# dexmal/dexbotic

Hardware: AMD Instinct MI355X
Metric: episodes/sec DB-CogACT fine-tune (higher is better)
Workload: dtype bf16; 1 GPU; DB-CogACT fine-tune step (CLIP-L/14@224 x1 view, Qwen2.5-7B-class 28L decoder, DiT-B head, AdamW), 16 episodes/GPU, 32-token instruction, S=287; global_batch=16, seq_len=287, parallelism=dp1, optimizer=AdamW serial, grad_accum=1, activations=resident

## Files before the change

dexbotic_amd/csrc/norm.hip:

```cpp
#include <stdlib.h>

#include "common.h"

namespace {

template <typename T, typename TW, int VEC>
__global__ __launch_bounds__(256) void rmsnorm_fwd_k(const T* __restrict__ x, const TW* __restrict__ w,
                                                     T* __restrict__ y, float* __restrict__ rstd_out,
                                                     int64_t rows, int64_t cols, float eps) {
  const int lane = threadIdx.x & 63;
  const int64_t row = (int64_t)blockIdx.x * 4 + (threadIdx.x >> 6);
  if (row >= rows) return;
  const T* xr = x + row * cols;
  float ss = 0.f;
  for (int64_t c = (int64_t)lane * VEC; c < cols; c += 64 * VEC) {
    float v[VEC];
    Vec<T, VEC>::ld(v, xr + c);
#pragma unroll
    for (int i = 0; i < VEC; ++i) ss += v[i] * v[i];
  }
  ss = wave_sum(ss);
  const float rstd = rsqrtf(ss / (float)cols + eps);
  if (lane == 0 && rstd_out) rstd_out[row] = rstd;
  T* yr = y + row * cols;
// ... 192 lines not shown
    if (slab) {
      for (int turn = 0; turn < 4; ++turn) {
        if (turn == wave && ok) {
          const T* xr = x + row * cols;
          const T* x2r = ADD ? x2 + row * cols : nullptr;
          const T* gr = dy + row * cols;
          for (int64_t c = (int64_t)lane * VEC; c < cols; c += 64 * VEC) {
            float xv[VEC], gv[VEC];
            ld_row<T, VEC, ADD>(xv, xr, x2r, c);
            Vec<T, VEC>::ld(gv, gr + c);
#pragma unroll
            for (int i = 0; i < VEC; ++i) {
              slab[c + i] += gv[i] * ((xv[i] - mu) * rs);
              slab[cols + c + i] += gv[i];
            }
          }
        }
        __syncthreads();
      }
    }
  }
}

template <typename T, bool DIRECT = false>
__global__ __launch_bounds__(256) void colsum_stage1_k(const T* __restrict__ x, int64_t ld, float* __restrict__ part,
                                                       int64_t rows, int64_t cols, int vec, int accumulate = 0) {
  __shared__ float red[4][256];
  const int lane = threadIdx.x & 63, wave = threadIdx.x >> 6;
  const int64_t c0 = (int64_t)blockIdx.x * 256 + lane * 4;
  const int64_t per = (rows + gridDim.y - 1) / gridDim.y;
  const int64_t r0 = (int64_t)blockIdx.y * per, r1 = min(rows, r0 + per);
  float a[4] = {0.f, 0.f, 0.f, 0.f};
  if (c0 < cols) {
    const int n_ok = (int)min((int64_t)4, cols - c0);
    for (int64_t r = r0 + wave; r < r1; r += 4) {
      const T* p = x + r * ld + c0;
      if (vec && n_ok == 4) {
        float v[4];
        Vec<T, 4>::ld(v, p);
#pragma unroll
        for (int i = 0; i < 4; ++i) a[i] += v[i];
      } else {
        for (int i = 0; i < n_ok; ++i) a[i] += ldf<T>(p + i);
      }
    }
  }
#pragma unroll
  for (int i = 0; i < 4; ++i) red[wave][lane * 4 + i] = a[i];
  __syncthreads();
  const int t = threadIdx.x;
  const int64_t c = (int64_t)blockIdx.x * 256 + t;
  if (c < cols) {
    const float sum = red[0][t] + red[1][t] + red[2][t] + red[3][t];
    if (DIRECT) part[c] = accumulate ? part[c] + sum : sum;
    else part[(int64_t)blockIdx.y * cols + c] = sum;
  }
}
__global__ void colsum_stage2_k(const float* __restrict__ part, float* __restrict__ out, int nsplit, int64_t cols,
                                int accumulate) {
  const int64_t c = (int64_t)blockIdx.x * blockDim.x + threadIdx.x;
  if (c >= cols) return;
  float s = 0.f;
  int i = 0;
  for (; i + 8 <= nsplit; i += 8) {
    float v[8];
#pragma unroll
    for (int u = 0; u < 8; ++u) v[u] = part[(int64_t)(i + u) * cols + c];
#pragma unroll
    for (int u = 0; u < 8; ++u) s += v[u];
  }
  for (; i < nsplit; ++i) s += part[(int64_t)i * cols + c];
  out[c] = accumulate ? out[c] + s : s;
}

template <typename T>
__global__ __launch_bounds__(256) void colsum_fused_k(const T* __restrict__ x, int64_t ld, float* __restrict__ part,
                                                      float* __restrict__ out, int64_t rows, int64_t cols, int vec,
                                                      int accumulate, int* __restrict__ cnt) {
  __shared__ float red[4][256];
  __shared__ int last;
  const int lane = threadIdx.x & 63, wave = threadIdx.x >> 6;
  const int64_t c0 = (int64_t)blockIdx.x * 256 + lane * 4;
  const int64_t per = (rows + gridDim.y - 1) / gridDim.y;
  const int64_t r0 = (int64_t)blockIdx.y * per, r1 = min(rows, r0 + per);
  float a[4] = {0.f, 0.f, 0.f, 0.f};
  if (c0 < cols) {
    const int n_ok = (int)min((int64_t)4, cols - c0);
    for (int64_t r = r0 + wave; r < r1; r += 4) {
      const T* p = x + r * ld + c0;
      if (vec && n_ok == 4) {
        float v[4];
        Vec<T, 4>::ld(v, p);
#pragma unroll
        for (int i = 0; i < 4; ++i) a[i] += v[i];
      } else {
        for (int i = 0; i < n_ok; ++i) a[i] += ldf<T>(p + i);
      }
    }
  }
#pragma unroll
  for (int i = 0; i < 4; ++i) red[wave][lane * 4 + i] = a[i];
  __syncthreads();
  const int t = threadIdx.x;
  const int64_t c = (int64_t)blockIdx.x * 256 + t;
  if (c < cols)
    __hip_atomic_store(part + (int64_t)blockIdx.y * cols + c, red[0][t] + red[1][t] + red[2][t] + red[3][t], __ATOMIC_RELAXED,
                       __HIP_MEMORY_SCOPE_AGENT);
  asm volatile("s_waitcnt vmcnt(0)" ::: "memory");
  __syncthreads();
  if (t == 0) {
    const int arrived = __hip_atomic_fetch_add(cnt + blockIdx.x, 1, __ATOMIC_RELAXED, __HIP_MEMORY_SCOPE_AGENT) + 1;
    last = arrived == (int)gridDim.y;
    if (last) __hip_atomic_store(cnt + blockIdx.x, 0, __ATOMIC_RELAXED, __HIP_MEMORY_SCOPE_AGENT);
  }
  __syncthreads();
  if (!last || c >= cols) return;
  const int nsplit = (int)gridDim.y;
  float s = 0.f;
  int i = 0;
  for (; i + 8 <= nsplit; i += 8) {
    float v[8];
#pragma unroll
    for (int u = 0; u < 8; ++u) v[u] = __hip_atomic_load(part + (int64_t)(i + u) * cols + c, __ATOMIC_RELAXED, __HIP_MEMORY_SCOPE_AGENT);
#pragma unroll
    for (int u = 0; u < 8; ++u) s += v[u];
  }
  for (; i < nsplit; ++i) s += __hip_atomic_load(part + (int64_t)i * cols + c, __ATOMIC_RELAXED, __HIP_MEMORY_SCOPE_AGENT);
  out[c] = accumulate ? out[c] + s : s;
}

inline bool al16(const void* p) { return (reinterpret_cast<uintptr_t>(p) & 15) == 0; }
inline bool al8(const void* p) { return (reinterpret_cast<uintptr_t>(p) & 7) == 0; }

template <typename T, typename TW, bool LN>
__global__ __launch_bounds__(256) void norm_bwd_fast_k(const T* __restrict__ dy, const T* __restrict__ x,
                                                       const TW* __restrict__ w, const float* __restrict__ mean,
                                                       const float* __restrict__ rstd, T* __restrict__ dx,
                                                       const T* __restrict__ res, float* __restrict__ partial,
                                                       int64_t rows, int64_t cols) {
  constexpr int NIT = 16;
  const int lane = threadIdx.x & 63, wave = threadIdx.x >> 6;
  const int64_t prow = (int64_t)blockIdx.x * 4 + wave;
  float aw[NIT][4], ab[NIT][4];
#pragma unroll
  for (int it = 0; it < NIT; ++it)
#pragma unroll
    for (int i = 0; i < 4; ++i) { aw[it][i] = 0.f; ab[it][i] = 0.f; }
  for (int64_t row = prow; row < rows; row += (int64_t)gridDim.x * 4) {
    const float rs = rstd[row];
    const float mu = LN ? mean[row] : 0.f;
    const T* xr = x + row * cols;
// ... 64 lines not shown
          }
        }
      }
      __syncthreads();
    }
    if (wave == 0) {
      float* pr = partial + (int64_t)blockIdx.x * (LN ? 2 : 1) * cols;
#pragma unroll
      for (int it = 0; it < NIT; ++it) {
        const int64_t c = ((int64_t)it * 64 + lane) * 4;
        if (c < cols) {
          const float4 t = *reinterpret_cast<const float4*>(sh + c);
          *reinterpret_cast<float4*>(pr + c) = make_float4(t.x + aw[it][0], t.y + aw[it][1], t.z + aw[it][2], t.w + aw[it][3]);
          if (LN) {
            const float4 u = *reinterpret_cast<const float4*>(sh + cols + c);
            *reinterpret_cast<float4*>(pr + cols + c) = make_float4(u.x + ab[it][0], u.y + ab[it][1], u.z + ab[it][2], u.w + ab[it][3]);
          }
        }
      }
    }
  }
}

template <typename TW, bool LN>
__global__ __launch_bounds__(256) void norm_bwd_fast8_k(const bf16_t* __restrict__ dy, const bf16_t* __restrict__ x,
                                                        const TW* __restrict__ w, const float* __restrict__ mean,
                                                        const float* __restrict__ rstd, bf16_t* __restrict__ dx,
                                                        const bf16_t* __restrict__ res, float* __restrict__ partial,
                                                        int64_t rows, int64_t cols) {
  constexpr int NIT = 8;
  typedef uint32_t u32x4 __attribute__((ext_vector_type(4)));
  const int lane = threadIdx.x & 63, wave = threadIdx.x >> 6;
  const int64_t prow = (int64_t)blockIdx.x * 4 + wave;
  float aw[NIT][8], ab[LN ? NIT : 1][8];
#pragma unroll
  for (int it = 0; it < NIT; ++it)
#pragma unroll
    for (int i = 0; i < 8; ++i) { aw[it][i] = 0.f; if (LN) ab[it][i] = 0.f; }
  auto unpack = [](const u32x4& v, float (&o)[8]) {
#pragma unroll
    for (int e = 0; e < 4; ++e) { o[2 * e] = __uint_as_float(v[e] << 16); o[2 * e + 1] = __uint_as_float(v[e] & 0xffff0000u); }
  };
  for (int64_t row = prow; row < rows; row += (int64_t)gridDim.x * 4) {
    const float rs = rstd[row];
    const float mu = LN ? mean[row] : 0.f;
    const bf16_t* xr = x + row * cols;
    const bf16_t* gr = dy + row * cols;
    u32x4 xv[NIT], gv[NIT];
#pragma unroll
    for (int it = 0; it < NIT; ++it) {
      const int64_t c = ((int64_t)it * 64 + lane) * 8;
      xv[it] = c < cols ? *reinterpret_cast<const u32x4*>(xr + c) : (u32x4){0u, 0u, 0u, 0u};
      gv[it] = c < cols ? *reinterpret_cast<const u32x4*>(gr + c) : (u32x4){0u, 0u, 0u, 0u};
    }
    float s1 = 0.f, s2 = 0.f;
#pragma unroll
    for (int it = 0; it < NIT; ++it) {
      const int64_t c = ((int64_t)it * 64 + lane) * 8;
      if (c < cols) {
        float xf[8], gf[8], w0[4] = {1.f, 1.f, 1.f, 1.f}, w1[4] = {1.f, 1.f, 1.f, 1.f};
        unpack(xv[it], xf); unpack(gv[it], gf);
        if (w) { Vec<TW, 4>::ld(w0, w + c); Vec<TW, 4>::ld(w1, w + c + 4); }
#pragma unroll
        for (int i = 0; i < 8; ++i) {
          const float g = gf[i] * (i < 4 ? w0[i] : w1[i - 4]);
          s1 += g;
          s2 += g * ((xf[i] - mu) * rs);
        }
      }
    }
    const float c1 = LN ? wave_sum(s1) / (float)cols : 0.f;
    const float c2 = wave_sum(s2) / (float)cols;
    bf16_t* dxr = dx + row * cols;
#pragma unroll
    for (int it = 0; it < NIT; ++it) {
      const int64_t c = ((int64_t)it * 64 + lane) * 8;
      if (c < cols) {
        float xf[8], gf[8], o[8], w0[4] = {1.f, 1.f, 1.f, 1.f}, w1[4] = {1.f, 1.f, 1.f, 1.f};
        unpack(xv[it], xf); unpack(gv[it], gf);
        if (w) { Vec<TW, 4>::ld(w0, w + c); Vec<TW, 4>::ld(w1, w + c + 4); }
#pragma unroll
        for (int i = 0; i < 8; ++i) {
          const float xh = (xf[i] - mu) * rs;
          o[i] = rs * (gf[i] * (i < 4 ? w0[i] : w1[i - 4]) - c1 - xh * c2);
          aw[it][i] += gf[i] * (LN ? xh : rnd<bf16_t>(xh));
          if (LN) ab[it][i] += gf[i];
        }
        if (res) {
          float rf[8];
          unpack(*reinterpret_cast<const u32x4*>(res + row * cols + c), rf);
#pragma unroll
          for (int i = 0; i < 8; ++i) o[i] += rf[i];
        }
        u32x4 ov;
#pragma unroll
        for (int e = 0; e < 4; ++e) ov[e] = pack_bf16x2(o[2 * e], o[2 * e + 1]);
        *reinterpret_cast<u32x4*>(dxr + c) = ov;
      }
    }
  }
  if (partial) {
    __shared__ float sh[(LN ? 2 : 1) * 4096];
    for (int turn = 3; turn >= 1; --turn) {
      if (wave == turn) {
#pragma unroll
        for (int it = 0; it < NIT; ++it) {
          const int64_t c = ((int64_t)it * 64 + lane) * 8;
          if (c < cols) {
#pragma unroll
            for (int i = 0; i < 8; ++i) {
              sh[c + i] = turn == 3 ? aw[it][i] : sh[c + i] + aw[it][i];
              if (LN) sh[cols + c + i] = turn == 3 ? ab[it][i] : sh[cols + c + i] + ab[it][i];
            }
          }
        }
      }
      __syncthreads();
    }
    if (wave == 0) {
      float* pr = partial + (int64_t)blockIdx.x * (LN ? 2 : 1) * cols;
#pragma unroll
      for (int it = 0; it < NIT; ++it) {
        const int64_t c = ((int64_t)it * 64 + lane) * 8;
        if (c < cols) {
#pragma unroll
// ... 119 lines not shown
      }
    }
  }
}

constexpr int NORM_BWD_MAX_BLOCKS = 512;
constexpr int64_t NORM_BWD_FAST_MAX_COLS = 4096;

template <bool LN>
bool launch_norm_bwd_fast(const void* dy, const void* x, const void* w, const float* mean, const float* rstd, void* dx,
                          const void* res, float* partial, int64_t rows, int64_t cols, int dtype, int w_dtype, bool vec_ok, hipStream_t st) {
  int64_t g = (rows + 3) / 4;
  if (g > NORM_BWD_MAX_BLOCKS) g = NORM_BWD_MAX_BLOCKS;
  dim3 grid((unsigned)g);
  if (!LN && vec_ok && dtype == DXA_BF16 && cols % 16 == 0 && cols <= 8192 && (cols * 4) % 16 == 0 &&
      (!partial || (reinterpret_cast<uintptr_t>(partial) & 15) == 0)) {
#define LAUNCH_SPLIT(TW_, NIT_, NS_) hipLaunchKernelGGL((rmsnorm_bwd_split_k<TW_, NIT_, NS_>), grid, dim3(NS_ * 128), 0, st, (const bf16_t*)dy, (const bf16_t*)x, (const TW_*)w, rstd, (bf16_t*)dx, (const bf16_t*)res, partial, rows, cols)
    if (w_dtype == DXA_BF16) { if (cols > 4096) LAUNCH_SPLIT(bf16_t, 8, 4); else LAUNCH_SPLIT(bf16_t, 4, 4); }
    else { if (cols > 4096) LAUNCH_SPLIT(float, 8, 4); else LAUNCH_SPLIT(float, 4, 4); }
#undef LAUNCH_SPLIT
    return true;
  }
  if (!vec_ok || cols % 4 != 0 || cols > NORM_BWD_FAST_MAX_COLS) return false;
  if (dtype == DXA_BF16 && cols % 8 == 0 && !LN) {
    if (w_dtype == DXA_BF16)
      hipLaunchKernelGGL((norm_bwd_fast8_k<bf16_t, LN>), grid, dim3(256), 0, st, (const bf16_t*)dy, (const bf16_t*)x, (const bf16_t*)w, mean, rstd, (bf16_t*)dx, (const bf16_t*)res, partial, rows, cols);
    else
      hipLaunchKernelGGL((norm_bwd_fast8_k<float, LN>), grid, dim3(256), 0, st, (const bf16_t*)dy, (const bf16_t*)x, (const float*)w, mean, rstd, (bf16_t*)dx, (const bf16_t*)res, partial, rows, cols);
    return true;
  }
  if (dtype == DXA_BF16 && w_dtype == DXA_BF16)
    hipLaunchKernelGGL((norm_bwd_fast_k<bf16_t, bf16_t, LN>), grid, dim3(256), 0, st, (const bf16_t*)dy, (const bf16_t*)x, (const bf16_t*)w, mean, rstd, (bf16_t*)dx, (const bf16_t*)res, partial, rows, cols);
  else if (dtype == DXA_BF16)
    hipLaunchKernelGGL((norm_bwd_fast_k<bf16_t, float, LN>), grid, dim3(256), 0, st, (const bf16_t*)dy, (const bf16_t*)x, (const float*)w, mean, rstd, (bf16_t*)dx, (const bf16_t*)res, partial, rows, cols);
  else
    hipLaunchKernelGGL((norm_bwd_fast_k<float, float, LN>), grid, dim3(256), 0, st, (const float*)dy, (const float*)x, (const float*)w, mean, rstd, (float*)dx, (const float*)res, partial, rows, cols);
  return true;
}

}

extern "C" int dxa_norm_bwd_blocks(int64_t rows) {
  int64_t g = (rows + 3) / 4;
  if (g < 1) g = 1;
  if (g > NORM_BWD_MAX_BLOCKS) g = NORM_BWD_MAX_BLOCKS;
  return (int)g;
}

static int check_norm_dtypes(int dtype, int w_dtype, const char* who) {
  if (!(dtype == DXA_F32 || dtype == DXA_BF16) || !(w_dtype == DXA_F32 || w_dtype == DXA_BF16) ||
      (dtype == DXA_F32 && w_dtype == DXA_BF16)) {
// ... 32 lines not shown
  const float rstd = rsqrtf(ss / (float)cols + eps);
  if (lane == 0 && rstd_out) rstd_out[row] = rstd;
  bf16_t* yr = y + row * cols;
#pragma unroll
  for (int it = 0; it < NIT; ++it) {
    const int64_t c = ((int64_t)it * 64 + lane) * 8;
    if (c < cols) {
      float g0[4] = {1.f, 1.f, 1.f, 1.f}, g1[4] = {1.f, 1.f, 1.f, 1.f};
      if (w) {
        Vec<TW, 4>::ld(g0, w + c);
        Vec<TW, 4>::ld(g1, w + c + 4);
      }
      const float g[8] = {g0[0], g0[1], g0[2], g0[3], g1[0], g1[1], g1[2], g1[3]};
      u32x4 o;
#pragma unroll
      for (int e = 0; e < 4; ++e) {
        const float a = __uint_as_float(v[it][e] << 16), b = __uint_as_float(v[it][e] & 0xffff0000u);
        o[e] = pack_bf16x2(g[2 * e] * rnd<bf16_t>(a * rstd), g[2 * e + 1] * rnd<bf16_t>(b * rstd));
      }
      *reinterpret_cast<u32x4*>(yr + c) = o;
    }
  }
}
}

extern "C" int dxa_rmsnorm_fwd(const void* x, const void* w, void* y, float* rstd, int64_t rows, int64_t cols,
                               float eps, int dtype, int w_dtype, dxa_stream_t stream) {
  if (int rc = check_norm_dtypes(dtype, w_dtype, "dxa_rmsnorm_fwd")) return rc;
  DXA_CHECK_ARG(x && y && rows >= 0 && cols > 0, "dxa_rmsnorm_fwd: bad args");
  if (rows == 0) return DXA_OK;
  hipStream_t st = (hipStream_t)stream;
  const bool vec_ok = al16(x) && al16(y) && (!w || al16(w));
  dim3 grid((unsigned)((rows + 3) / 4));
  if (dtype == DXA_BF16 && vec_ok && cols % 8 == 0 && cols <= 8192) {
    if (w_dtype == DXA_BF16) hipLaunchKernelGGL((rmsnorm_fwd_fast_k<bf16_t>), grid, dim3(256), 0, st, (const bf16_t*)x, (const bf16_t*)w, (bf16_t*)y, rstd, rows, cols, eps);
    else hipLaunchKernelGGL((rmsnorm_fwd_fast_k<float>), grid, dim3(256), 0, st, (const bf16_t*)x, (const float*)w, (bf16_t*)y, rstd, rows, cols, eps);
    DXA_CHECK_LAUNCH();
    return DXA_OK;
  }
  if (dtype == DXA_BF16 && w_dtype == DXA_BF16) {
    if (vec_ok && cols % 4 == 0) hipLaunchKernelGGL((rmsnorm_fwd_k<bf16_t, bf16_t, 4>), grid, dim3(256), 0, st, (const bf16_t*)x, (const bf16_t*)w, (bf16_t*)y, rstd, rows, cols, eps);
    else hipLaunchKernelGGL((rmsnorm_fwd_k<bf16_t, bf16_t, 1>), grid, dim3(256), 0, st, (const bf16_t*)x, (const bf16_t*)w, (bf16_t*)y, rstd, rows, cols, eps);
  } else if (dtype == DXA_BF16) {
    if (vec_ok && cols % 4 == 0) hipLaunchKernelGGL((rmsnorm_fwd_k<bf16_t, float, 4>), grid, dim3(256), 0, st, (const bf16_t*)x, (const float*)w, (bf16_t*)y, rstd, rows, cols, eps);
    else hipLaunchKernelGGL((rmsnorm_fwd_k<bf16_t, float, 1>), grid, dim3(256), 0, st, (const bf16_t*)x, (const float*)w, (bf16_t*)y, rstd, rows, cols, eps);
  } else {
// ... 21 lines not shown
  if (dtype == DXA_BF16 && w_dtype == DXA_BF16) {
    if (vec_ok && cols % 4 == 0) hipLaunchKernelGGL((rmsnorm_bwd_k<bf16_t, bf16_t, 4>), grid, dim3(256), 0, st, (const bf16_t*)dy, (const bf16_t*)x, (const bf16_t*)w, rstd, (bf16_t*)dx, (const bf16_t*)residual, partial_dw, rows, cols);
    else hipLaunchKernelGGL((rmsnorm_bwd_k<bf16_t, bf16_t, 1>), grid, dim3(256), 0, st, (const bf16_t*)dy, (const bf16_t*)x, (const bf16_t*)w, rstd, (bf16_t*)dx, (const bf16_t*)residual, partial_dw, rows, cols);
  } else if (dtype == DXA_BF16) {
    if (vec_ok && cols % 4 == 0) hipLaunchKernelGGL((rmsnorm_bwd_k<bf16_t, float, 4>), grid, dim3(256), 0, st, (const bf16_t*)dy, (const bf16_t*)x, (const float*)w, rstd, (bf16_t*)dx, (const bf16_t*)residual, partial_dw, rows, cols);
    else hipLaunchKernelGGL((rmsnorm_bwd_k<bf16_t, float, 1>), grid, dim3(256), 0, st, (const bf16_t*)dy, (const bf16_t*)x, (const float*)w, rstd, (bf16_t*)dx, (const bf16_t*)residual, partial_dw, rows, cols);
  } else {
    if (vec_ok && cols % 4 == 0) hipLaunchKernelGGL((rmsnorm_bwd_k<float, float, 4>), grid, dim3(256), 0, st, (const float*)dy, (const float*)x, (const float*)w, rstd, (float*)dx, (const float*)residual, partial_dw, rows, cols);
    else hipLaunchKernelGGL((rmsnorm_bwd_k<float, float, 1>), grid, dim3(256), 0, st, (const float*)dy, (const float*)x, (const float*)w, rstd, (float*)dx, (const float*)residual, partial_dw, rows, cols);
  }
  DXA_CHECK_LAUNCH();
  return DXA_OK;
}

extern "C" int dxa_layernorm_fwd(const void* x, const void* w, const void* b, void* y, float* mean, float* rstd,
                                 int64_t rows, int64_t cols, float eps, int dtype, int w_dtype,
                                 dxa_stream_t stream) {
  if (int rc = check_norm_dtypes(dtype, w_dtype, "dxa_layernorm_fwd")) return rc;
  DXA_CHECK_ARG(x && y && rows >= 0 && cols > 0, "dxa_layernorm_fwd: bad args");
  if (rows == 0) return DXA_OK;
  hipStream_t st = (hipStream_t)stream;
  const bool vec_ok = al16(x) && al16(y) && (!w || al16(w)) && (!b || al16(b));
  dim3 grid((unsigned)((rows + 3) / 4));
  if (dtype == DXA_BF16 && w_dtype == DXA_BF16) {
    if (vec_ok && cols % 4 == 0) hipLaunchKernelGGL((layernorm_fwd_k<bf16_t, bf16_t, 4>), grid, dim3(256), 0, st, (const bf16_t*)x, (const bf16_t*)w, (const bf16_t*)b, (bf16_t*)y, mean, rstd, rows, cols, eps);
    else hipLaunchKernelGGL((layernorm_fwd_k<bf16_t, bf16_t, 1>), grid, dim3(256), 0, st, (const bf16_t*)x, (const bf16_t*)w, (const bf16_t*)b, (bf16_t*)y, mean, rstd, rows, cols, eps);
  } else if (dtype == DXA_BF16) {
    if (vec_ok && cols % 4 == 0) hipLaunchKernelGGL((layernorm_fwd_k<bf16_t, float, 4>), grid, dim3(256), 0, st, (const bf16_t*)x, (const float*)w, (const float*)b, (bf16_t*)y, mean, rstd, rows, cols, eps);
    else hipLaunchKernelGGL((layernorm_fwd_k<bf16_t, float, 1>), grid, dim3(256), 0, st, (const bf16_t*)x, (const float*)w, (const float*)b, (bf16_t*)y, mean, rstd, rows, cols, eps);
  } else {
    if (vec_ok && cols % 4 == 0) hipLaunchKernelGGL((layernorm_fwd_k<float, float, 4>), grid, dim3(256), 0, st, (const float*)x, (const float*)w, (const float*)b, (float*)y, mean, rstd, rows, cols, eps);
    else hipLaunchKernelGGL((layernorm_fwd_k<float, float, 1>), grid, dim3(256), 0, st, (const float*)x, (const float*)w, (const float*)b, (float*)y, mean, rstd, rows, cols, eps);
  }
  DXA_CHECK_LAUNCH();
  return DXA_OK;
}

extern "C" int dxa_layernorm_bwd(const void* dy, const void* x, const void* w, const float* mean,
                                 const float* rstd, void* dx, const void* residual, float* partial_dwdb, int64_t rows,
                                 int64_t cols, int dtype, int w_dtype, dxa_stream_t stream) {
  if (int rc = check_norm_dtypes(dtype, w_dtype, "dxa_layernorm_bwd")) return rc;
  DXA_CHECK_ARG(dy && x && mean && rstd && dx && rows >= 0 && cols > 0, "dxa_layernorm_bwd: bad args");
  DXA_CHECK_ARG(!w || partial_dwdb, "dxa_layernorm_bwd: partial_dwdb required when w is given");
  if (rows == 0) return DXA_OK;
  hipStream_t st = (hipStream_t)stream;
  const bool vec_ok = al16(x) && al16(dy) && al16(dx) && (!w || al16(w)) && (!partial_dwdb || al16(partial_dwdb)) && (!residual || al16(residual));
// ... 6 lines not shown
  if (dtype == DXA_BF16 && w_dtype == DXA_BF16) {
    if (vec_ok && cols % 4 == 0) hipLaunchKernelGGL((layernorm_bwd_k<bf16_t, bf16_t, 4>), grid, dim3(256), 0, st, (const bf16_t*)dy, (const bf16_t*)x, (const bf16_t*)w, mean, rstd, (bf16_t*)dx, (const bf16_t*)residual, part, rows, cols);
    else hipLaunchKernelGGL((layernorm_bwd_k<bf16_t, bf16_t, 1>), grid, dim3(256), 0, st, (const bf16_t*)dy, (const bf16_t*)x, (const bf16_t*)w, mean, rstd, (bf16_t*)dx, (const bf16_t*)residual, part, rows, cols);
  } else if (dtype == DXA_BF16) {
    if (vec_ok && cols % 4 == 0) hipLaunchKernelGGL((layernorm_bwd_k<bf16_t, float, 4>), grid, dim3(256), 0, st, (const bf16_t*)dy, (const bf16_t*)x, (const float*)w, mean, rstd, (bf16_t*)dx, (const bf16_t*)residual, part, rows, cols);
    else hipLaunchKernelGGL((layernorm_bwd_k<bf16_t, float, 1>), grid, dim3(256), 0, st, (const bf16_t*)dy, (const bf16_t*)x, (const float*)w, mean, rstd, (bf16_t*)dx, (const bf16_t*)residual, part, rows, cols);
  } else {
    if (vec_ok && cols % 4 == 0) hipLaunchKernelGGL((layernorm_bwd_k<float, float, 4>), grid, dim3(256), 0, st, (const float*)dy, (const float*)x, (const float*)w, mean, rstd, (float*)dx, (const float*)residual, part, rows, cols);
    else hipLaunchKernelGGL((layernorm_bwd_k<float, float, 1>), grid, dim3(256), 0, st, (const float*)dy, (const float*)x, (const float*)w, mean, rstd, (float*)dx, (const float*)residual, part, rows, cols);
  }
  DXA_CHECK_LAUNCH();
  return DXA_OK;
}

extern "C" int dxa_add_layernorm_fwd(const void* x, const void* res, const void* w, const void* b, void* y, float* mean,
                                     float* rstd, int64_t rows, int64_t cols, float eps, int dtype, int w_dtype,
                                     dxa_stream_t stream) {
  if (int rc = check_norm_dtypes(dtype, w_dtype, "dxa_add_layernorm_fwd")) return rc;
  DXA_CHECK_ARG(x && res && y, "dxa_add_layernorm_fwd: null x / res / y");
  DXA_CHECK_ARG(rows >= 0 && cols > 0, "dxa_add_layernorm_fwd: bad sizes (rows %lld, cols %lld)", (long long)rows, (long long)cols);
  if (rows == 0) return DXA_OK;
  hipStream_t st = (hipStream_t)stream;
  const bool vec = al16(x) && al16(res) && al16(y) && (!w || al16(w)) && (!b || al16(b)) && cols % 4 == 0;
  dim3 grid((unsigned)((rows + 3) / 4));
#define ADD_LN_FWD(T_, TW_, V_) hipLaunchKernelGGL((layernorm_fwd_k<T_, TW_, V_, true>), grid, dim3(256), 0, st, (const T_*)x, (const TW_*)w, (const TW_*)b, (T_*)y, mean, rstd, rows, cols, eps, (const T_*)res)
  if (dtype == DXA_BF16 && w_dtype == DXA_BF16) { if (vec) ADD_LN_FWD(bf16_t, bf16_t, 4); else ADD_LN_FWD(bf16_t, bf16_t, 1); }
  else if (dtype == DXA_BF16) { if (vec) ADD_LN_FWD(bf16_t, float, 4); else ADD_LN_FWD(bf16_t, float, 1); }
  else { if (vec) ADD_LN_FWD(float, float, 4); else ADD_LN_FWD(float, float, 1); }
#undef ADD_LN_FWD
  DXA_CHECK_LAUNCH();
  return DXA_OK;
}

extern "C" int dxa_add_layernorm_bwd(const void* dy, const void* x, const void* res, const void* w, const float* mean,
                                     const float* rstd, void* dx, float* partial_dwdb, int64_t rows, int64_t cols, int dtype,
                                     int w_dtype, dxa_stream_t stream) {
  if (int rc = check_norm_dtypes(dtype, w_dtype, "dxa_add_layernorm_bwd")) return rc;
  DXA_CHECK_ARG(dy && x && res && mean && rstd && dx, "dxa_add_layernorm_bwd: null dy / x / res / mean / rstd / dx");
  DXA_CHECK_ARG(rows >= 0 && cols > 0, "dxa_add_layernorm_bwd: bad sizes (rows %lld, cols %lld)", (long long)rows, (long long)cols);
  DXA_CHECK_ARG(!w || partial_dwdb, "dxa_add_layernorm_bwd: partial_dwdb required when w is given");
  if (rows == 0) return DXA_OK;
  hipStream_t st = (hipStream_t)stream;
  const bool vec = al16(x) && al16(res) && al16(dy) && al16(dx) && (!w || al16(w)) && cols % 4 == 0;
  dim3 grid((unsigned)dxa_norm_bwd_blocks(rows));
  float* part = w ? partial_dwdb : nullptr;
#define ADD_LN_BWD(T_, TW_, V_) hipLaunchKernelGGL((layernorm_bwd_k<T_, TW_, V_, true>), grid, dim3(256), 0, st, (const T_*)dy, (const T_*)x, (const TW_*)w, mean, rstd, (T_*)dx, (const T_*)nullptr, part, rows, cols, (const T_*)res)
  if (dtype == DXA_BF16 && w_dtype == DXA_BF16) { if (vec) ADD_LN_BWD(bf16_t, bf16_t, 4); else ADD_LN_BWD(bf16_t, bf16_t, 1); }
  else if (dtype == DXA_BF16) { if (vec) ADD_LN_BWD(bf16_t, float, 4); else ADD_LN_BWD(bf16_t, float, 1); }
  else { if (vec) ADD_LN_BWD(float, float, 4); else ADD_LN_BWD(float, float, 1); }
#undef ADD_LN_BWD
  DXA_CHECK_LAUNCH();
  return DXA_OK;
}

namespace {
constexpr int COLSUM_CNT = 4096;
StreamBlock colsum_counters(COLSUM_CNT * sizeof(int));
}

extern "C" int dxa_colsum(const void* x, int64_t ld, float* out, int64_t rows, int64_t cols, int dtype,
                          int accumulate, float* scratch, size_t scratch_bytes, dxa_stream_t stream) {
  DXA_CHECK_ARG(x && out && rows >= 0 && cols > 0 && ld >= cols, "dxa_colsum: bad args");
  DXA_CHECK_ARG(dtype == DXA_F32 || dtype == DXA_BF16, "dxa_colsum: bad dtype");
  hipStream_t st = (hipStream_t)stream;
  int nsplit = (int)((rows + 31) / 32);
  if (nsplit < 1) nsplit = 1;
  if (nsplit > 64) nsplit = 64;
  DXA_CHECK_ARG(scratch && scratch_bytes >= (size_t)nsplit * cols * sizeof(float),
                "dxa_colsum: scratch too small (need %zu bytes)", (size_t)nsplit * cols * sizeof(float));
  dim3 grid((unsigned)((cols + 255) / 256), (unsigned)nsplit);
  const size_t es = dtype == DXA_BF16 ? 2 : 4;
  const int vec = ((reinterpret_cast<uintptr_t>(x) % (4 * es)) == 0) && (ld % 4 == 0);
  if (rows <= 32) {
    dim3 g1((unsigned)((cols + 255) / 256), 1);
    if (dtype == DXA_BF16)
      hipLaunchKernelGGL((colsum_stage1_k<bf16_t, true>), g1, dim3(256), 0, st, (const bf16_t*)x, ld, out, rows, cols, vec, accumulate);
    else
      hipLaunchKernelGGL((colsum_stage1_k<float, true>), g1, dim3(256), 0, st, (const float*)x, ld, out, rows, cols, vec, accumulate);
    DXA_CHECK_LAUNCH();
    return DXA_OK;
  }
  int* cnt = nullptr;
  if (grid.x <= COLSUM_CNT) {
    if (int rc = colsum_counters.get(st, &cnt)) return rc;
  }
  if (cnt != nullptr) {
    if (dtype == DXA_BF16)
      hipLaunchKernelGGL((colsum_fused_k<bf16_t>), grid, dim3(256), 0, st, (const bf16_t*)x, ld, scratch, out, rows, cols, vec, accumulate, cnt);
    else
      hipLaunchKernelGGL((colsum_fused_k<float>), grid, dim3(256), 0, st, (const float*)x, ld, scratch, out, rows, cols, vec, accumulate, cnt);
    DXA_CHECK_LAUNCH();
    return DXA_OK;
  }
  if (dtype == DXA_BF16)
    hipLaunchKernelGGL((colsum_stage1_k<bf16_t>), grid, dim3(256), 0, st, (const bf16_t*)x, ld, scratch, rows, cols, vec);
  else
    hipLaunchKernelGGL((colsum_stage1_k<float>), grid, dim3(256), 0, st, (const float*)x, ld, scratch, rows, cols, vec);
  hipLaunchKernelGGL(colsum_stage2_k, dim3((unsigned)((cols + 63) / 64)), dim3(64), 0, st, scratch, out, nsplit,
                     cols, accumulate);
  DXA_CHECK_LAUNCH();
  return DXA_OK;
}

namespace {

template <typename TW, int VEC>
__device__ __forceinline__ void ld_w(float (&o)[VEC], const TW* p) {
  if constexpr (VEC == 8 && sizeof(TW) == 4) {
    float a[4], b[4];
    Vec<float, 4>::ld(a, reinterpret_cast<const float*>(p));
    Vec<float, 4>::ld(b, reinterpret_cast<const float*>(p) + 4);
#pragma unroll
    for (int i = 0; i < 4; ++i) { o[i] = a[i]; o[4 + i] = b[i]; }
  } else {
    Vec<TW, VEC>::ld(o, p);
  }
}

__device__ __forceinline__ int64_t ds_quarter(int64_t row, int q, int G, int h, int C) {
  const int64_t n = row / ((int64_t)h * h);
  const int o = (int)(row - n * h * h);
  const int j = o / h, i = o - j * h;
// ... 626 lines not shown
```

Before: 70.93 episodes/s.

## Widen colsum loads, add fast bf16 LayerNorm fwd, extend fast8 norm bwd to LN

The column-sum kernels now load 16 bytes per lane (8 bf16 per lane), keep several row loads in flight at once, and run the final reduction with more unrolling. The split count is recomputed so no split gets an empty row range. A new register-resident bf16 LayerNorm forward kernel (plain and residual-add variants) is templated on how many 512-column chunks each wave holds. The 8-wide norm backward kernel is templated on column count, keeps norm weights in registers for small widths, prefetches the residual, and now also handles LayerNorm. These changes target memory bandwidth and latency in the normalization and bias-gradient kernels, at the cost of more template instantiations and higher register pressure.

Result: no change. 71.34 episodes/s, median of 6 (+0.6%).

```diff
diff --git a/dexbotic_amd/csrc/norm.hip b/dexbotic_amd/csrc/norm.hip
--- a/dexbotic_amd/csrc/norm.hip
+++ b/dexbotic_amd/csrc/norm.hip
@@ -238,111 +238,153 @@
   }
 }
 
+constexpr int COLSUM_G = 8;
+
+template <typename T, int MODE>
+__device__ __forceinline__ void colsum_ld(float (&v)[16 / sizeof(T)], const T* p, int n_ok) {
+  constexpr int VW = 16 / sizeof(T);
+  if constexpr (MODE == 2) {
+    Vec<T, VW>::ld(v, p);
+  } else if constexpr (MODE == 1) {
+    float lo[4], hi[4];
+    Vec<T, 4>::ld(lo, p);
+    Vec<T, 4>::ld(hi, p + 4);
+#pragma unroll
+    for (int i = 0; i < 4; ++i) { v[i] = lo[i]; v[4 + i] = hi[i]; }
+  } else {
+#pragma unroll
+    for (int i = 0; i < VW; ++i) {
+      const float e = ldf<T>(p + min(i, n_ok - 1));
+      v[i] = i < n_ok ? e : 0.f;
+    }
+  }
+}
+
+template <typename T, int MODE>
+__device__ __forceinline__ void colsum_rows(float (&a)[16 / sizeof(T)], const T* __restrict__ xw, int64_t pitch, int n, int64_t c0,
+                                            int n_ok) {
+  constexpr int VW = 16 / sizeof(T);
+  for (int k = 0; k < n; k += COLSUM_G) {
+    float v[COLSUM_G][VW];
+#pragma unroll
+    for (int u = 0; u < COLSUM_G; ++u) colsum_ld<T, MODE>(v[u], xw + (int64_t)min(k + u, n - 1) * pitch + c0, n_ok);
+#pragma unroll
+    for (int u = 0; u < COLSUM_G; ++u) {
+      const uint32_t live = k + u < n ? 0xffffffffu : 0u;
+#pragma unroll
+      for (int i = 0; i < VW; ++i) a[i] += __uint_as_float(__float_as_uint(v[u][i]) & live);
+    }
+  }
+}
+
+template <typename T>
+__device__ __forceinline__ void colsum_tile(const T* __restrict__ x, int64_t ld, int64_t rows, int64_t cols, int mode,
+                                            float (*red)[64 * (16 / sizeof(T))]) {
+  constexpr int VW = 16 / sizeof(T);
+  const int lane = threadIdx.x & 63, wave = __builtin_amdgcn_readfirstlane(threadIdx.x >> 6);
+  const int64_t c0 = (int64_t)blockIdx.x * (64 * VW) + lane * VW;
+  const int64_t per = (rows + gridDim.y - 1) / gridDim.y;
+  const int64_t r0 = (int64_t)blockIdx.y * per + wave, r1 = min(rows, (int64_t)blockIdx.y * per + per);
+  const int n = r0 < r1 ? (int)((r1 - r0 + 3) / 4) : 0;
+  float a[VW];
+#pragma unroll
+  for (int i = 0; i < VW; ++i) a[i] = 0.f;
+  if (c0 < cols) {
+    const int n_ok = (int)min((int64_t)VW, cols - c0);
+    const T* xw = x + r0 * ld;
+    if (mode == 2 && n_ok == VW) colsum_rows<T, 2>(a, xw, 4 * ld, n, c0, n_ok);
+    else if (sizeof(T) == 2 && mode == 1 && n_ok == VW) colsum_rows<T, (sizeof(T) == 2 ? 1 : 0)>(a, xw, 4 * ld, n, c0, n_ok);
+    else colsum_rows<T, 0>(a, xw, 4 * ld, n, c0, n_ok);
+  }
+#pragma unroll
+  for (int i = 0; i < VW; ++i) red[wave][lane * VW + i] = a[i];
+  __syncthreads();
+}
+
+template <int TILE, bool COHERENT, int G>
+__device__ __forceinline__ void colsum_fold_g(const float* __restrict__ part, int nsplit, int64_t cols, float* __restrict__ out,
+                                              int accumulate) {
+  constexpr int NC = TILE / 256;
+  const int64_t c0 = (int64_t)blockIdx.x * TILE + threadIdx.x;
+  if (c0 >= cols) return;
+  int64_t c[NC];
+#pragma unroll
+  for (int j = 0; j < NC; ++j) c[j] = min(c0 + j * 256, cols - 1);
+  float s[NC];
+#pragma unroll
+  for (int j = 0; j < NC; ++j) s[j] = 0.f;
+  for (int i = 0; i < nsplit; i += G) {
+    float v[NC][G];
+#pragma unroll
+    for (int u = 0; u < G; ++u)
+#pragma unroll
+      for (int j = 0; j < NC; ++j) {
+        const float* q = part + (int64_t)min(i + u, nsplit - 1) * cols + c[j];
+        v[j][u] = COHERENT ? __hip_atomic_load(q, __ATOMIC_RELAXED, __HIP_MEMORY_SCOPE_AGENT) : *q;
+      }
+#pragma unroll
+    for (int u = 0; u < G; ++u) {
+      const uint32_t live = i + u < nsplit ? 0xffffffffu : 0u;
+#pragma unroll
+      for (int j = 0; j < NC; ++j) s[j] += __uint_as_float(__float_as_uint(v[j][u]) & live);
+    }
+  }
+#pragma unroll
+  for (int j = 0; j < NC; ++j)
+    if (c0 + j * 256 < cols) out[c[j]] = accumulate ? out[c[j]] + s[j] : s[j];
+}
+template <int TILE, bool COHERENT>
+__device__ __forceinline__ void colsum_fold(const float* __restrict__ part, int nsplit, int64_t cols, float* __restrict__ out,
+                                            int accumulate) {
+  if (nsplit <= 16) colsum_fold_g<TILE, COHERENT, 16>(part, nsplit, cols, out, accumulate);
+  else if (nsplit <= 32) colsum_fold_g<TILE, COHERENT, 32>(part, nsplit, cols, out, accumulate);
+  else if (nsplit <= 48) colsum_fold_g<TILE, COHERENT, 48>(part, nsplit, cols, out, accumulate);
+  else colsum_fold_g<TILE, COHERENT, 64>(part, nsplit, cols, out, accumulate);
+}
+
 template <typename T, bool DIRECT = false>
 __global__ __launch_bounds__(256) void colsum_stage1_k(const T* __restrict__ x, int64_t ld, float* __restrict__ part,
-                                                       int64_t rows, int64_t cols, int vec, int accumulate = 0) {
-  __shared__ float red[4][256];
-  const int lane = threadIdx.x & 63, wave = threadIdx.x >> 6;
-  const int64_t c0 = (int64_t)blockIdx.x * 256 + lane * 4;
-  const int64_t per = (rows + gridDim.y - 1) / gridDim.y;
-  const int64_t r0 = (int64_t)blockIdx.y * per, r1 = min(rows, r0 + per);
-  float a[4] = {0.f, 0.f, 0.f, 0.f};
-  if (c0 < cols) {
-    const int n_ok = (int)min((int64_t)4, cols - c0);
-    for (int64_t r = r0 + wave; r < r1; r += 4) {
-      const T* p = x + r * ld + c0;
-      if (vec && n_ok == 4) {
-        float v[4];
-        Vec<T, 4>::ld(v, p);
-#pragma unroll
-        for (int i = 0; i < 4; ++i) a[i] += v[i];
-      } else {
-        for (int i = 0; i < n_ok; ++i) a[i] += ldf<T>(p + i);
-      }
-    }
-  }
-#pragma unroll
-  for (int i = 0; i < 4; ++i) red[wave][lane * 4 + i] = a[i];
-  __syncthreads();
-  const int t = threadIdx.x;
-  const int64_t c = (int64_t)blockIdx.x * 256 + t;
-  if (c < cols) {
+                                                       int64_t rows, int64_t cols, int mode, int accumulate = 0) {
+  constexpr int TILE = 64 * (16 / sizeof(T));
+  __shared__ float red[4][TILE];
+  colsum_tile<T>(x, ld, rows, cols, mode, red);
+  for (int t = threadIdx.x; t < TILE; t += 256) {
+    const int64_t c = (int64_t)blockIdx.x * TILE + t;
+    if (c >= cols) break;
     const float sum = red[0][t] + red[1][t] + red[2][t] + red[3][t];
     if (DIRECT) part[c] = accumulate ? part[c] + sum : sum;
     else part[(int64_t)blockIdx.y * cols + c] = sum;
   }
 }
-__global__ void colsum_stage2_k(const float* __restrict__ part, float* __restrict__ out, int nsplit, int64_t cols,
-                                int accumulate) {
-  const int64_t c = (int64_t)blockIdx.x * blockDim.x + threadIdx.x;
-  if (c >= cols) return;
-  float s = 0.f;
-  int i = 0;
-  for (; i + 8 <= nsplit; i += 8) {
-    float v[8];
-#pragma unroll
-    for (int u = 0; u < 8; ++u) v[u] = part[(int64_t)(i + u) * cols + c];
-#pragma unroll
-    for (int u = 0; u < 8; ++u) s += v[u];
-  }
-  for (; i < nsplit; ++i) s += part[(int64_t)i * cols + c];
-  out[c] = accumulate ? out[c] + s : s;
+template <int TILE>
+__global__ __launch_bounds__(256) void colsum_stage2_k(const float* __restrict__ part, float* __restrict__ out, int nsplit,
+                                                       int64_t cols, int accumulate) {
+  colsum_fold<TILE, false>(part, nsplit, cols, out, accumulate);
 }
 
 template <typename T>
 __global__ __launch_bounds__(256) void colsum_fused_k(const T* __restrict__ x, int64_t ld, float* __restrict__ part,
-                                                      float* __restrict__ out, int64_t rows, int64_t cols, int vec,
+                                                      float* __restrict__ out, int64_t rows, int64_t cols, int mode,
                                                       int accumulate, int* __restrict__ cnt) {
-  __shared__ float red[4][256];
+  constexpr int TILE = 64 * (16 / sizeof(T));
+  __shared__ float red[4][TILE];
   __shared__ int last;
-  const int lane = threadIdx.x & 63, wave = threadIdx.x >> 6;
-  const int64_t c0 = (int64_t)blockIdx.x * 256 + lane * 4;
-  const int64_t per = (rows + gridDim.y - 1) / gridDim.y;
-  const int64_t r0 = (int64_t)blockIdx.y * per, r1 = min(rows, r0 + per);
-  float a[4] = {0.f, 0.f, 0.f, 0.f};
-  if (c0 < cols) {
-    const int n_ok = (int)min((int64_t)4, cols - c0);
-    for (int64_t r = r0 + wave; r < r1; r += 4) {
-      const T* p = x + r * ld + c0;
-      if (vec && n_ok == 4) {
-        float v[4];
-        Vec<T, 4>::ld(v, p);
-#pragma unroll
-        for (int i = 0; i < 4; ++i) a[i] += v[i];
-      } else {
-        for (int i = 0; i < n_ok; ++i) a[i] += ldf<T>(p + i);
-      }
-    }
-  }
-#pragma unroll
-  for (int i = 0; i < 4; ++i) red[wave][lane * 4 + i] = a[i];
-  __syncthreads();
-  const int t = threadIdx.x;
-  const int64_t c = (int64_t)blockIdx.x * 256 + t;
-  if (c < cols)
+  colsum_tile<T>(x, ld, rows, cols, mode, red);
+  for (int t = threadIdx.x; t < TILE; t += 256) {
+    const int64_t c = (int64_t)blockIdx.x * TILE + t;
+    if (c >= cols) break;
     __hip_atomic_store(part + (int64_t)blockIdx.y * cols + c, red[0][t] + red[1][t] + red[2][t] + red[3][t], __ATOMIC_RELAXED,
                        __HIP_MEMORY_SCOPE_AGENT);
+  }
   asm volatile("s_waitcnt vmcnt(0)" ::: "memory");
   __syncthreads();
-  if (t == 0) {
+  if (threadIdx.x == 0) {
     const int arrived = __hip_atomic_fetch_add(cnt + blockIdx.x, 1, __ATOMIC_RELAXED, __HIP_MEMORY_SCOPE_AGENT) + 1;
     last = arrived == (int)gridDim.y;
     if (last) __hip_atomic_store(cnt + blockIdx.x, 0, __ATOMIC_RELAXED, __HIP_MEMORY_SCOPE_AGENT);
   }
   __syncthreads();
-  if (!last || c >= cols) return;
-  const int nsplit = (int)gridDim.y;
-  float s = 0.f;
-  int i = 0;
-  for (; i + 8 <= nsplit; i += 8) {
-    float v[8];
-#pragma unroll
-    for (int u = 0; u < 8; ++u) v[u] = __hip_atomic_load(part + (int64_t)(i + u) * cols + c, __ATOMIC_RELAXED, __HIP_MEMORY_SCOPE_AGENT);
-#pragma unroll
-    for (int u = 0; u < 8; ++u) s += v[u];
-  }
-  for (; i < nsplit; ++i) s += __hip_atomic_load(part + (int64_t)i * cols + c, __ATOMIC_RELAXED, __HIP_MEMORY_SCOPE_AGENT);
-  out[c] = accumulate ? out[c] + s : s;
+  if (last) colsum_fold<TILE, true>(part, (int)gridDim.y, cols, out, accumulate);
 }
 
 inline bool al16(const void* p) { return (reinterpret_cast<uintptr_t>(p) & 15) == 0; }
@@ -453,17 +495,17 @@
   }
 }
 
-template <typename TW, bool LN>
+template <typename TW, bool LN, int NIT>
 __global__ __launch_bounds__(256) void norm_bwd_fast8_k(const bf16_t* __restrict__ dy, const bf16_t* __restrict__ x,
                                                         const TW* __restrict__ w, const float* __restrict__ mean,
                                                         const float* __restrict__ rstd, bf16_t* __restrict__ dx,
                                                         const bf16_t* __restrict__ res, float* __restrict__ partial,
                                                         int64_t rows, int64_t cols) {
-  constexpr int NIT = 8;
+  constexpr bool HOIST = NIT <= 4;
   typedef uint32_t u32x4 __attribute__((ext_vector_type(4)));
   const int lane = threadIdx.x & 63, wave = threadIdx.x >> 6;
   const int64_t prow = (int64_t)blockIdx.x * 4 + wave;
-  float aw[NIT][8], ab[LN ? NIT : 1][8];
+  float aw[NIT][8], ab[LN ? NIT : 1][8], wh[HOIST ? NIT : 1][8];
 #pragma unroll
   for (int it = 0; it < NIT; ++it)
 #pragma unroll
@@ -472,29 +514,44 @@
 #pragma unroll
     for (int e = 0; e < 4; ++e) { o[2 * e] = __uint_as_float(v[e] << 16); o[2 * e + 1] = __uint_as_float(v[e] & 0xffff0000u); }
   };
+  auto ld_w = [&](float (&o)[8], int64_t c) {
+    float w0[4] = {1.f, 1.f, 1.f, 1.f}, w1[4] = {1.f, 1.f, 1.f, 1.f};
+    if (w) { Vec<TW, 4>::ld(w0, w + c); Vec<TW, 4>::ld(w1, w + c + 4); }
+#pragma unroll
+    for (int i = 0; i < 4; ++i) { o[i] = w0[i]; o[4 + i] = w1[i]; }
+  };
+  if (HOIST) {
+#pragma unroll
+    for (int it = 0; it < NIT; ++it) {
+      const int64_t c = ((int64_t)it * 64 + lane) * 8;
+      if (c < cols) ld_w(wh[it], c);
+    }
+  }
   for (int64_t row = prow; row < rows; row += (int64_t)gridDim.x * 4) {
     const float rs = rstd[row];
     const float mu = LN ? mean[row] : 0.f;
-    const bf16_t* xr = x + row * cols;
-    const bf16_t* gr = dy + row * cols;
-    u32x4 xv[NIT], gv[NIT];
+    const int64_t ro = row * cols;
+    u32x4 xv[NIT], gv[NIT], rv[NIT];
 #pragma unroll
     for (int it = 0; it < NIT; ++it) {
       const int64_t c = ((int64_t)it * 64 + lane) * 8;
-      xv[it] = c < cols ? *reinterpret_cast<const u32x4*>(xr + c) : (u32x4){0u, 0u, 0u, 0u};
-      gv[it] = c < cols ? *reinterpret_cast<const u32x4*>(gr + c) : (u32x4){0u, 0u, 0u, 0u};
+      const bool in = c < cols;
+      xv[it] = in ? *reinterpret_cast<const u32x4*>(x + ro + c) : (u32x4){0u, 0u, 0u, 0u};
+      gv[it] = in ? *reinterpret_cast<const u32x4*>(dy + ro + c) : (u32x4){0u, 0u, 0u, 0u};
+      rv[it] = (in && res) ? *reinterpret_cast<const u32x4*>(res + ro + c) : (u32x4){0u, 0u, 0u, 0u};
     }
     float s1 = 0.f, s2 = 0.f;
 #pragma unroll
     for (int it = 0; it < NIT; ++it) {
       const int64_t c = ((int64_t)it * 64 + lane) * 8;
       if (c < cols) {
-        float xf[8], gf[8], w0[4] = {1.f, 1.f, 1.f, 1.f}, w1[4] = {1.f, 1.f, 1.f, 1.f};
+        float xf[8], gf[8], wl[8];
         unpack(xv[it], xf); unpack(gv[it], gf);
-        if (w) { Vec<TW, 4>::ld(w0, w + c); Vec<TW, 4>::ld(w1, w + c + 4); }
+        if (!HOIST) ld_w(wl, c);
+        const float (&wf)[8] = HOIST ? wh[HOIST ? it : 0] : wl;
 #pragma unroll
         for (int i = 0; i < 8; ++i) {
-          const float g = gf[i] * (i < 4 ? w0[i] : w1[i - 4]);
+          const float g = gf[i] * wf[i];
           s1 += g;
           s2 += g * ((xf[i] - mu) * rs);
         }
@@ -502,36 +559,36 @@
     }
     const float c1 = LN ? wave_sum(s1) / (float)cols : 0.f;
     const float c2 = wave_sum(s2) / (float)cols;
-    bf16_t* dxr = dx + row * cols;
 #pragma unroll
     for (int it = 0; it < NIT; ++it) {
       const int64_t c = ((int64_t)it * 64 + lane) * 8;
       if (c < cols) {
-        float xf[8], gf[8], o[8], w0[4] = {1.f, 1.f, 1.f, 1.f}, w1[4] = {1.f, 1.f, 1.f, 1.f};
+        float xf[8], gf[8], o[8], wl[8];
         unpack(xv[it], xf); unpack(gv[it], gf);
-        if (w) { Vec<TW, 4>::ld(w0, w + c); Vec<TW, 4>::ld(w1, w + c + 4); }
+        if (!HOIST) ld_w(wl, c);
+        const float (&wf)[8] = HOIST ? wh[HOIST ? it : 0] : wl;
 #pragma unroll
         for (int i = 0; i < 8; ++i) {
           const float xh = (xf[i] - mu) * rs;
-          o[i] = rs * (gf[i] * (i < 4 ? w0[i] : w1[i - 4]) - c1 - xh * c2);
+          o[i] = rs * (gf[i] * wf[i] - c1 - xh * c2);
           aw[it][i] += gf[i] * (LN ? xh : rnd<bf16_t>(xh));
           if (LN) ab[it][i] += gf[i];
         }
         if (res) {
           float rf[8];
-          unpack(*reinterpret_cast<const u32x4*>(res + row * cols + c), rf);
+          unpack(rv[it], rf);
 #pragma unroll
           for (int i = 0; i < 8; ++i) o[i] += rf[i];
         }
         u32x4 ov;
 #pragma unroll
         for (int e = 0; e < 4; ++e) ov[e] = pack_bf16x2(o[2 * e], o[2 * e + 1]);
-        *reinterpret_cast<u32x4*>(dxr + c) = ov;
+        *reinterpret_cast<u32x4*>(dx + ro + c) = ov;
       }
     }
   }
   if (partial) {
-    __shared__ float sh[(LN ? 2 : 1) * 4096];
+    __shared__ float sh[(LN ? 2 : 1) * NIT * 512];
     for (int turn = 3; turn >= 1; --turn) {
       if (wave == turn) {
 #pragma unroll
@@ -697,11 +754,15 @@
     return true;
   }
   if (!vec_ok || cols % 4 != 0 || cols > NORM_BWD_FAST_MAX_COLS) return false;
-  if (dtype == DXA_BF16 && cols % 8 == 0 && !LN) {
-    if (w_dtype == DXA_BF16)
-      hipLaunchKernelGGL((norm_bwd_fast8_k<bf16_t, LN>), grid, dim3(256), 0, st, (const bf16_t*)dy, (const bf16_t*)x, (const bf16_t*)w, mean, rstd, (bf16_t*)dx, (const bf16_t*)res, partial, rows, cols);
-    else
-      hipLaunchKernelGGL((norm_bwd_fast8_k<float, LN>), grid, dim3(256), 0, st, (const bf16_t*)dy, (const bf16_t*)x, (const float*)w, mean, rstd, (bf16_t*)dx, (const bf16_t*)res, partial, rows, cols);
+  if (dtype == DXA_BF16 && cols % 8 == 0) {
+#define LAUNCH_FAST8(TW_, NIT_) hipLaunchKernelGGL((norm_bwd_fast8_k<TW_, LN, NIT_>), grid, dim3(256), 0, st, (const bf16_t*)dy, (const bf16_t*)x, (const TW_*)w, mean, rstd, (bf16_t*)dx, (const bf16_t*)res, partial, rows, cols)
+#define LAUNCH_FAST8_W(NIT_) do { if (w_dtype == DXA_BF16) LAUNCH_FAST8(bf16_t, NIT_); else LAUNCH_FAST8(float, NIT_); } while (0)
+    if (cols <= 512) LAUNCH_FAST8_W(1);
+    else if (cols <= 1024) LAUNCH_FAST8_W(2);
+    else if (cols <= 2048) LAUNCH_FAST8_W(4);
+    else LAUNCH_FAST8_W(8);
+#undef LAUNCH_FAST8_W
+#undef LAUNCH_FAST8
     return true;
   }
   if (dtype == DXA_BF16 && w_dtype == DXA_BF16)
@@ -780,6 +841,138 @@
     }
   }
 }
+
+template <typename TW> struct Raw8;
+template <> struct Raw8<float> {
+  float4 a, b;
+  __device__ __forceinline__ void ld(const float* p) { a = *reinterpret_cast<const float4*>(p); b = *reinterpret_cast<const float4*>(p + 4); }
+  __device__ __forceinline__ void get(float (&o)[8]) const { o[0] = a.x; o[1] = a.y; o[2] = a.z; o[3] = a.w; o[4] = b.x; o[5] = b.y; o[6] = b.z; o[7] = b.w; }
+};
+template <> struct Raw8<bf16_t> {
+  uint4 v;
+  __device__ __forceinline__ void ld(const bf16_t* p) { v = *reinterpret_cast<const uint4*>(p); }
+  __device__ __forceinline__ void get(float (&o)[8]) const {
+    o[0] = __uint_as_float(v.x << 16); o[1] = __uint_as_float(v.x & 0xffff0000u); o[2] = __uint_as_float(v.y << 16); o[3] = __uint_as_float(v.y & 0xffff0000u);
+    o[4] = __uint_as_float(v.z << 16); o[5] = __uint_as_float(v.z & 0xffff0000u); o[6] = __uint_as_float(v.w << 16); o[7] = __uint_as_float(v.w & 0xffff0000u);
+  }
+};
+
+template <typename TW, int NIT, bool ADD>
+__global__ __launch_bounds__(256) void layernorm_fwd_fast_k(const bf16_t* __restrict__ x, const TW* __restrict__ w,
+                                                            const TW* __restrict__ b, bf16_t* __restrict__ y,
+                                                            float* __restrict__ mean_out, float* __restrict__ rstd_out,
+                                                            int64_t rows, int64_t cols, float eps, const bf16_t* __restrict__ x2) {
+  constexpr bool EARLY = NIT <= 4;
+  typedef uint32_t u32x4 __attribute__((ext_vector_type(4)));
+  const int lane = threadIdx.x & 63;
+  const int64_t row = (int64_t)blockIdx.x * 4 + (threadIdx.x >> 6);
+  if (row >= rows) return;
+  const bf16_t* xr = x + row * cols;
+  u32x4 v[NIT], v2[ADD ? NIT : 1];
+  Raw8<TW> wr[EARLY ? NIT : 1], br[EARLY ? NIT : 1];
+#pragma unroll
+  for (int it = 0; it < NIT; ++it) {
+    const int64_t c = ((int64_t)it * 64 + lane) * 8;
+    v[it] = *reinterpret_cast<const u32x4*>(xr + (c < cols ? c : 0));
+    if (ADD) v2[ADD ? it : 0] = *reinterpret_cast<const u32x4*>(x2 + row * cols + (c < cols ? c : 0));
+  }
+  if (EARLY) {
+#pragma unroll
+    for (int it = 0; it < NIT; ++it) {
+      const int64_t c = ((int64_t)it * 64 + lane) * 8;
+      if (w) wr[EARLY ? it : 0].ld(w + (c < cols ? c : 0));
+      if (b) br[EARLY ? it : 0].ld(b + (c < cols ? c : 0));
+    }
+  }
+#pragma unroll
+  for (int it = 0; it < NIT; ++it) {
+    const int64_t c = ((int64_t)it * 64 + lane) * 8;
+    if (c >= cols) {
+      v[it] = (u32x4){0u, 0u, 0u, 0u};
+      if (ADD) v2[ADD ? it : 0] = (u32x4){0u, 0u, 0u, 0u};
+    }
+  }
+  auto chunk = [&](int it, float (&o)[8]) {
+#pragma unroll
+    for (int e = 0; e < 4; ++e) { o[2 * e] = __uint_as_float(v[it][e] << 16); o[2 * e + 1] = __uint_as_float(v[it][e] & 0xffff0000u); }
+    if (ADD) {
+      const u32x4& t = v2[ADD ? it : 0];
+#pragma unroll
+      for (int e = 0; e < 4; ++e) { o[2 * e] += __uint_as_float(t[e] << 16); o[2 * e + 1] += __uint_as_float(t[e] & 0xffff0000u); }
+    }
+  };
+  float s = 0.f;
+#pragma unroll
+  for (int it = 0; it < NIT; ++it) {
+    float xf[8];
+    chunk(it, xf);
+#pragma unroll
+    for (int e = 0; e < 4; ++e) s += xf[2 * e] + xf[2 * e + 1];
+  }
+  const float mean = wave_sum(s) / (float)cols;
+  float ss = 0.f;
+#pragma unroll
+  for (int it = 0; it < NIT; ++it) {
+    const int64_t c = ((int64_t)it * 64 + lane) * 8;
+    if (c < cols) {
+      float xf[8];
+      chunk(it, xf);
+#pragma unroll
+      for (int e = 0; e < 4; ++e) {
+        const float d0 = xf[2 * e] - mean, d1 = xf[2 * e + 1] - mean;
+        ss += d0 * d0 + d1 * d1;
+      }
+    }
+  }
+  const float rstd = rsqrtf(wave_sum(ss) / (float)cols + eps);
+  if (lane == 0) {
+    if (mean_out) mean_out[row] = mean;
+    if (rstd_out) rstd_out[row] = rstd;
+  }
+  bf16_t* yr = y + row * cols;
+#pragma unroll
+  for (int it = 0; it < NIT; ++it) {
+    const int64_t c = ((int64_t)it * 64 + lane) * 8;
+    if (c < cols) {
+      float g[8], bb[8], xf[8];
+      if (EARLY) {
+        wr[EARLY ? it : 0].get(g);
+        br[EARLY ? it : 0].get(bb);
+      } else {
+        Raw8<TW> wl, bl;
+        if (w) wl.ld(w + c);
+        if (b) bl.ld(b + c);
+        wl.get(g);
+        bl.get(bb);
+      }
+#pragma unroll
+      for (int i = 0; i < 8; ++i) { g[i] = w ? g[i] : 1.f; bb[i] = b ? bb[i] : 0.f; }
+      chunk(it, xf);
+      u32x4 o;
+#pragma unroll
+      for (int e = 0; e < 4; ++e)
+        o[e] = pack_bf16x2((xf[2 * e] - mean) * rstd * g[2 * e] + bb[2 * e], (xf[2 * e + 1] - mean) * rstd * g[2 * e + 1] + bb[2 * e + 1]);
+      *reinterpret_cast<u32x4*>(yr + c) = o;
+    }
+  }
+}
+
+template <bool ADD>
+bool launch_layernorm_fwd_fast(const void* x, const void* x2, const void* w, const void* b, void* y, float* mean, float* rstd,
+                               int64_t rows, int64_t cols, float eps, int dtype, int w_dtype, bool al_ok, hipStream_t st) {
+  if (dtype != DXA_BF16 || !al_ok || cols % 8 != 0 || cols > 8192) return false;
+  dim3 grid((unsigned)((rows + 3) / 4));
+#define LN_FWD_FAST(TW_, NIT_) hipLaunchKernelGGL((layernorm_fwd_fast_k<TW_, NIT_, ADD>), grid, dim3(256), 0, st, (const bf16_t*)x, (const TW_*)w, (const TW_*)b, (bf16_t*)y, mean, rstd, rows, cols, eps, (const bf16_t*)x2)
+#define LN_FWD_FAST_W(NIT_) do { if (w_dtype == DXA_BF16) LN_FWD_FAST(bf16_t, NIT_); else LN_FWD_FAST(float, NIT_); } while (0)
+  if (cols <= 512) LN_FWD_FAST_W(1);
+  else if (cols <= 1024) LN_FWD_FAST_W(2);
+  else if (cols <= 2048) LN_FWD_FAST_W(4);
+  else if (cols <= 4096) LN_FWD_FAST_W(8);
+  else LN_FWD_FAST_W(16);
+#undef LN_FWD_FAST_W
+#undef LN_FWD_FAST
+  return true;
+}
 }
 
 extern "C" int dxa_rmsnorm_fwd(const void* x, const void* w, void* y, float* rstd, int64_t rows, int64_t cols,
@@ -847,6 +1040,10 @@
   hipStream_t st = (hipStream_t)stream;
   const bool vec_ok = al16(x) && al16(y) && (!w || al16(w)) && (!b || al16(b));
   dim3 grid((unsigned)((rows + 3) / 4));
+  if (launch_layernorm_fwd_fast<false>(x, nullptr, w, b, y, mean, rstd, rows, cols, eps, dtype, w_dtype, vec_ok, st)) {
+    DXA_CHECK_LAUNCH();
+    return DXA_OK;
+  }
   if (dtype == DXA_BF16 && w_dtype == DXA_BF16) {
     if (vec_ok && cols % 4 == 0) hipLaunchKernelGGL((layernorm_fwd_k<bf16_t, bf16_t, 4>), grid, dim3(256), 0, st, (const bf16_t*)x, (const bf16_t*)w, (const bf16_t*)b, (bf16_t*)y, mean, rstd, rows, cols, eps);
     else hipLaunchKernelGGL((layernorm_fwd_k<bf16_t, bf16_t, 1>), grid, dim3(256), 0, st, (const bf16_t*)x, (const bf16_t*)w, (const bf16_t*)b, (bf16_t*)y, mean, rstd, rows, cols, eps);
@@ -899,6 +1096,10 @@
   if (rows == 0) return DXA_OK;
   hipStream_t st = (hipStream_t)stream;
   const bool vec = al16(x) && al16(res) && al16(y) && (!w || al16(w)) && (!b || al16(b)) && cols % 4 == 0;
+  if (launch_layernorm_fwd_fast<true>(x, res, w, b, y, mean, rstd, rows, cols, eps, dtype, w_dtype, vec, st)) {
+    DXA_CHECK_LAUNCH();
+    return DXA_OK;
+  }
   dim3 grid((unsigned)((rows + 3) / 4));
 #define ADD_LN_FWD(T_, TW_, V_) hipLaunchKernelGGL((layernorm_fwd_k<T_, TW_, V_, true>), grid, dim3(256), 0, st, (const T_*)x, (const TW_*)w, (const TW_*)b, (T_*)y, mean, rstd, rows, cols, eps, (const T_*)res)
   if (dtype == DXA_BF16 && w_dtype == DXA_BF16) { if (vec) ADD_LN_FWD(bf16_t, bf16_t, 4); else ADD_LN_FWD(bf16_t, bf16_t, 1); }
@@ -945,15 +1146,21 @@
   if (nsplit > 64) nsplit = 64;
   DXA_CHECK_ARG(scratch && scratch_bytes >= (size_t)nsplit * cols * sizeof(float),
                 "dxa_colsum: scratch too small (need %zu bytes)", (size_t)nsplit * cols * sizeof(float));
-  dim3 grid((unsigned)((cols + 255) / 256), (unsigned)nsplit);
+  if (rows > 0) {
+    const int64_t per = (rows + nsplit - 1) / nsplit;
+    nsplit = (int)((rows + per - 1) / per);
+  }
   const size_t es = dtype == DXA_BF16 ? 2 : 4;
-  const int vec = ((reinterpret_cast<uintptr_t>(x) % (4 * es)) == 0) && (ld % 4 == 0);
+  const int64_t tile = 64 * (16 / (int64_t)es);
+  dim3 grid((unsigned)((cols + tile - 1) / tile), (unsigned)nsplit);
+  const uintptr_t xa = reinterpret_cast<uintptr_t>(x);
+  const int mode = (xa % 16 == 0 && (ld * es) % 16 == 0) ? 2 : (dtype == DXA_BF16 && xa % 8 == 0 && ld % 4 == 0) ? 1 : 0;
   if (rows <= 32) {
-    dim3 g1((unsigned)((cols + 255) / 256), 1);
+    dim3 g1(grid.x, 1);
     if (dtype == DXA_BF16)
-      hipLaunchKernelGGL((colsum_stage1_k<bf16_t, true>), g1, dim3(256), 0, st, (const bf16_t*)x, ld, out, rows, cols, vec, accumulate);
+      hipLaunchKernelGGL((colsum_stage1_k<bf16_t, true>), g1, dim3(256), 0, st, (const bf16_t*)x, ld, out, rows, cols, mode, accumulate);
     else
-      hipLaunchKernelGGL((colsum_stage1_k<float, true>), g1, dim3(256), 0, st, (const float*)x, ld, out, rows, cols, vec, accumulate);
+      hipLaunchKernelGGL((colsum_stage1_k<float, true>), g1, dim3(256), 0, st, (const float*)x, ld, out, rows, cols, mode, accumulate);
     DXA_CHECK_LAUNCH();
     return DXA_OK;
   }
@@ -963,18 +1170,18 @@
   }
   if (cnt != nullptr) {
     if (dtype == DXA_BF16)
-      hipLaunchKernelGGL((colsum_fused_k<bf16_t>), grid, dim3(256), 0, st, (const bf16_t*)x, ld, scratch, out, rows, cols, vec, accumulate, cnt);
+      hipLaunchKernelGGL((colsum_fused_k<bf16_t>), grid, dim3(256), 0, st, (const bf16_t*)x, ld, scratch, out, rows, cols, mode, accumulate, cnt);
     else
-      hipLaunchKernelGGL((colsum_fused_k<float>), grid, dim3(256), 0, st, (const float*)x, ld, scratch, out, rows, cols, vec, accumulate, cnt);
+      hipLaunchKernelGGL((colsum_fused_k<float>), grid, dim3(256), 0, st, (const float*)x, ld, scratch, out, rows, cols, mode, accumulate, cnt);
     DXA_CHECK_LAUNCH();
     return DXA_OK;
   }
   if (dtype == DXA_BF16)
-    hipLaunchKernelGGL((colsum_stage1_k<bf16_t>), grid, dim3(256), 0, st, (const bf16_t*)x, ld, scratch, rows, cols, vec);
+    hipLaunchKernelGGL((colsum_stage1_k<bf16_t>), grid, dim3(256), 0, st, (const bf16_t*)x, ld, scratch, rows, cols, mode);
   else
-    hipLaunchKernelGGL((colsum_stage1_k<float>), grid, dim3(256), 0, st, (const float*)x, ld, scratch, rows, cols, vec);
-  hipLaunchKernelGGL(colsum_stage2_k, dim3((unsigned)((cols + 63) / 64)), dim3(64), 0, st, scratch, out, nsplit,
-                     cols, accumulate);
+    hipLaunchKernelGGL((colsum_stage1_k<float>), grid, dim3(256), 0, st, (const float*)x, ld, scratch, rows, cols, mode);
+  if (dtype == DXA_BF16) hipLaunchKernelGGL(colsum_stage2_k<512>, dim3(grid.x), dim3(256), 0, st, scratch, out, nsplit, cols, accumulate);
+  else hipLaunchKernelGGL(colsum_stage2_k<256>, dim3(grid.x), dim3(256), 0, st, scratch, out, nsplit, cols, accumulate);
   DXA_CHECK_LAUNCH();
   return DXA_OK;
 }
```
